# pletzer/nemoflux

Measured on AMD Instinct MI355X. Metric: edge-flux integrals/sec, higher is better.
Workload: dtype f64

## Files before the change

### nemoflux_amd/csrc/nf_capi_field.hip

```cpp
#include "nf_capi.h"

using namespace nf;

static int g_batch_steps = 1;
static long g_batch_cellsteps = 32l << 20;
static int g_partial_full = 0;
static int g_use_graph = 1;
static int g_inner_signed = 1;
static int g_k3_pairs = 1;
static long g_knob_version = 0;

namespace nf {
int field_tuning_set(const char *name, int value)
{
    ++g_knob_version;
    if (!strcmp(name, "batch_steps")) {
        g_batch_steps = value;
        return NF_OK;
    }
    if (!strcmp(name, "batch_cellsteps_m")) {
        if (!(value >= 0 && value <= 2047)) return -1;
        g_batch_cellsteps = (long)value << 20;
        return NF_OK;
    }
    if (!strcmp(name, "partial_step_planes")) {
        g_partial_full = value != 0;
        return NF_OK;
    }
    if (!strcmp(name, "graph")) {
        g_use_graph = value != 0;
        return NF_OK;
    }
    if (!strcmp(name, "pass_inner_signed")) {
        g_inner_signed = value != 0;
        return NF_OK;
    }
    if (!strcmp(name, "pass_k3_pairs")) {
        g_k3_pairs = value != 0;
        return NF_OK;
    }
    return -1;
}
}

struct nf_field {
    hipStream_t stream = nullptr;
    long ny = 0, nx = 0, ncell = 0, nz = 0, nt = 0;
    struct Geometry {
        DevArray<double> xy, arc4, arcE, arcN;
        DevArray<unsigned long long> box;
        DevArray<double> iV;
        DevArray<double> abs;
        DevArray<double> aos;
        DevArray<double> uv2;
        DevArray<double> tr_planes;
        DevArray<unsigned long long> maxbits;
        DevArray<double> iVb, absb, scratchb;
        DevArray<int> zr;
        long batch_steps = 0, batch_version = -1;
    } geo;
    double box[4] = {0, 0, 0, 0};
    DevArray<double> thick;
    const void *u = nullptr, *v = nullptr;
    int uv_dtype = NF_F64, uv_on_device = 1;
    double fill = std::numeric_limits<double>::quiet_NaN();
    double fill2 = std::numeric_limits<double>::quiet_NaN();
    DevArray<char> stage_u, stage_v;
    int sverdrup = 0;
    long s_begin = 0, s_end = -1;
    int compact = 0;
    bool derived_stale = false;
    std::vector<std::vector<double>> polylines;
    std::vector<int> poly_cc;
    std::vector<int> tr_off;
    WeightSet ws;
    bool weights_built = false;
    int skip_unsupported = 0;
// ... 103 lines not shown
}

static int field_timed_k3_end(nf_field *f)
{
    if (!f->timing || f->ev_used == 0 || f->ev_dropped) return NF_OK;
    auto &t = f->ev[f->ev_used - 1];
    NF_HIP(hipEventRecord(t.e2, f->stream));
    t.has_k3 = true;
    return NF_OK;
}

static int field_ensure_derived(nf_field *f)
{
    if (!f->derived_stale) return NF_OK;
    NF_TRY(launch_expand_planes(f->geo.iV.get(), f->geo.abs.get(), f->ncell, f->ny, f->nx, f->stream));
    f->derived_stale = false;
    return NF_OK;
}

static int field_row_length(const nf_field *f) { return f->ws.nseg + (int)f->polylines.size(); }

struct StepForm {
    bool inner = false;
    bool to_uv2 = false;
};

static int field_step_input(nf_field *f, long t, int z0, int z1, const void **ut, const void **vt)
{
    const size_t es = elem_size(f->uv_dtype);
    const size_t step_bytes = (size_t)f->nz * f->ncell * es;
    if (f->uv_on_device) {
        *ut = (const char *)f->u + (size_t)t * step_bytes;
        *vt = (const char *)f->v + (size_t)t * step_bytes;
        return NF_OK;
    }
    NF_TRY(f->stage_u.reserve(step_bytes));
    NF_TRY(f->stage_v.reserve(step_bytes));
    const size_t off = (size_t)z0 * f->ncell * es, len = (size_t)(z1 - z0) * f->ncell * es;
    NF_HIP(hipMemcpyAsync(f->stage_u.get() + off, (const char *)f->u + (size_t)t * step_bytes + off, len,
                          hipMemcpyHostToDevice, f->stream));
    NF_HIP(hipMemcpyAsync(f->stage_v.get() + off, (const char *)f->v + (size_t)t * step_bytes + off, len,
                          hipMemcpyHostToDevice, f->stream));
    *ut = f->stage_u.get();
    *vt = f->stage_v.get();
    return NF_OK;
}

// ... 11 lines not shown
        if (row_dev && rowlen > 0) NF_HIP(hipMemsetAsync(row_dev, 0, sizeof(double) * rowlen, f->stream));
        return NF_OK;
    }
    const int z0 = (int)(lo - t * f->nz), z1 = (int)(hi - t * f->nz);
    const void *ut, *vt;
    NF_TRY(field_step_input(f, t, z0, z1, &ut, &vt));
    FluxArgs a{};
    a.u = ut;
    a.v = vt;
    a.dtype = f->uv_dtype;
    a.ncell = f->ncell;
    a.ny = f->ny;
    a.nx = f->nx;
    a.z0 = z0;
    a.z1 = z1;
    a.thickness = f->thick.get();
    a.arcE = f->geo.arcE.get();
    a.arcN = f->geo.arcN.get();
    a.fill = f->fill;
    a.fill2 = f->fill2;
    a.scale = kEarthRadiusSv / 1.e6;
    a.sverdrup = f->sverdrup;
    a.iV = f->geo.iV.get();
    if (form.to_uv2) a.iV = f->geo.uv2.get() - f->ncell;
    a.absU = f->geo.abs.get();
    a.absV = f->geo.abs.get() + f->ncell;
    a.maxbits = f->geo.maxbits.get();
    const bool partial = (z0 > 0 || z1 < (int)f->nz) && !g_partial_full;
    a.signed_only = (f->compact || partial || form.inner) && flux_supports_signed_only(a);
    NF_REQUIRE(!form.to_uv2 || a.signed_only, NF_ERR_STATE, "compute: a step into the second planes must be signed-only");
    if (!form.to_uv2) f->derived_stale = a.signed_only != 0;
    if (f->timing) {
        NF_TRY(field_timed_flux(f, a));
    } else {
        NF_TRY(launch_flux(a, f->stream));
    }
    if (row_dev && rowlen > 0 && !form.to_uv2) {
        NF_REQUIRE(f->weights_built, NF_ERR_STATE, "compute: build_weights first");
        NF_TRY(launch_integral(f->ws, f->geo.iV.get(), f->ncell, 2, f->nx, f->tr_off_dev.get(), (int)f->polylines.size(),
                               f->scratch.get(), row_dev, f->stream));
        NF_TRY(field_timed_k3_end(f));
    }
    return NF_OK;
}

static int field_profile_async(nf_field *f, long t, double *prof_dev)
{
    NF_REQUIRE(f->geo.arcE.get() && f->thick.get() && f->u && f->v, NF_ERR_STATE,
               "compute_profile: set_bounds, set_thickness and set_uv first");
    NF_REQUIRE(f->weights_built, NF_ERR_STATE, "compute_profile: build_weights first");
    NF_REQUIRE(t >= 0 && t < f->nt, NF_ERR_ARG, "compute_profile: time index out of range");
    const int rowlen = field_row_length(f);
    if (rowlen == 0) return NF_OK;
    const long s_end = f->s_end < 0 ? f->nt * f->nz : f->s_end;
    long lo = t * f->nz, hi = (t + 1) * f->nz;
    if (lo < f->s_begin) lo = f->s_begin;
    if (hi > s_end) hi = s_end;
    if (hi < lo) hi = lo;
    const int z0 = (int)(lo - t * f->nz), z1 = (int)(hi - t * f->nz);
    if (z0 > 0) NF_HIP(hipMemsetAsync(prof_dev, 0, sizeof(double) * rowlen * (size_t)z0, f->stream));
// ... 61 lines not shown
    a.dtype = f->uv_dtype;
    a.ncell = f->ncell;
    a.ny = f->ny;
    a.nx = f->nx;
    a.z0 = z0;
    a.z1 = z1;
    a.thickness = f->thick.get();
    a.arcE = f->geo.arcE.get();
    a.arcN = f->geo.arcN.get();
    a.fill = f->fill;
    a.fill2 = f->fill2;
    a.tfill = f->tau_fill;
    a.tfill2 = f->tau_fill2;
    a.ref = f->tau_ref;
    a.wrap_x = f->tau_wrap;
    a.scale = kEarthRadiusSv / 1.e6;
    a.sverdrup = f->sverdrup;
    a.planes = f->geo.tr_planes.get();
    NF_TRY(launch_tracer_flux(a, f->stream));
    return launch_integral(f->ws, f->geo.tr_planes.get() - f->ncell, f->ncell, 2, f->nx, f->tr_off_dev.get(),
                           (int)f->polylines.size(), f->scratch.get(), row_dev, f->stream);
}

static int field_pair_async(nf_field *f, long t, double *rows_dev, bool last)
{
    const int rowlen = field_row_length(f);
    StepForm first, second;
    first.inner = first.to_uv2 = true;
    second.inner = g_inner_signed && !last;
    NF_TRY(field_step_async(f, t, nullptr, first));
    NF_TRY(field_step_async(f, t + 1, nullptr, second));
    NF_TRY(launch_integral_pair(f->ws, f->geo.uv2.get(), f->geo.iV.get() + f->ncell, f->ncell, f->nx, f->tr_off_dev.get(),
                                (int)f->polylines.size(), f->scratch.get(), rows_dev + (size_t)t * rowlen, rowlen, f->stream));
    NF_TRY(field_timed_k3_end(f));
    return NF_OK;
}

static long batch_cell_steps() { return g_batch_cellsteps; }

static bool field_can_batch(const nf_field *f)
{
    return g_batch_steps && f->uv_on_device && f->nt >= 2 && f->nt < 65536 && f->nt * f->ncell <= batch_cell_steps() &&
           f->ncell <= (1l << 20) && f->weights_built;
}

static bool field_pass_pairs(const nf_field *f)
{
    if (!g_k3_pairs || integral_uses_edges() || !f->geo.uv2.get() || !f->weights_built) return false;
    const size_t step_bytes = (size_t)f->nz * f->ncell * elem_size(f->uv_dtype);
    FluxArgs a{};
    a.u = f->uv_on_device ? f->u : nullptr;
    a.v = f->uv_on_device ? f->v : nullptr;
    a.dtype = f->uv_dtype;
    a.ncell = f->ncell;
    return flux_supports_signed_only(a) && (!f->uv_on_device || step_bytes % 16 == 0);
}

static int field_prepare_pass(nf_field *f)
{
    if (!g_k3_pairs || integral_uses_edges() || f->geo.uv2.get() || !f->geo.iV.get() || f->nz <= 0) return NF_OK;
    const long total = f->nt * f->nz;
    const long s_end = f->s_end < 0 ? total : std::min(f->s_end, total);
    if (s_end - std::min(f->s_begin, s_end) < 2 * f->nz) return NF_OK;
    NF_TRY(f->geo.uv2.alloc((size_t)f->ncell * 2));
    return NF_OK;
}

static int field_all_steps_direct(nf_field *f, double *rows_dev)
{
    const int rowlen = field_row_length(f);
    const long total = f->nt * f->nz;
    const long s_end = f->s_end < 0 ? total : std::min(f->s_end, total);
    const long s_begin = std::min(f->s_begin, s_end);
    const long ta = s_end > s_begin ? s_begin / f->nz : 0;
    const long tb = s_end > s_begin ? (s_end - 1) / f->nz + 1 : 0;
    if (rowlen > 0) {
        if (ta > 0) NF_HIP(hipMemsetAsync(rows_dev, 0, sizeof(double) * rowlen * (size_t)ta, f->stream));
        if (tb < f->nt)
            NF_HIP(hipMemsetAsync(rows_dev + (size_t)tb * rowlen, 0, sizeof(double) * rowlen * (size_t)(f->nt - tb),
                                  f->stream));
    }
    const long wa = (ta < tb && s_begin > ta * f->nz) ? ta + 1 : ta;
    const long wb = std::max(wa, (ta < tb && s_end < tb * f->nz) ? tb - 1 : tb);
    const bool pairs = field_pass_pairs(f) && rowlen > 0;
    const long pa = pairs ? wa + (wb - wa) % 2 : wb;
    for (long t = ta; t < tb;) {
        const bool last = t + 1 == tb;
        if (t >= pa && t + 1 < wb) {
            NF_TRY(field_pair_async(f, t, rows_dev, t + 2 == tb));
            t += 2;
        } else {
            StepForm form;
            form.inner = g_inner_signed && !last;
            NF_TRY(field_step_async(f, t, rows_dev + (size_t)t * rowlen, form));
            t += 1;
        }
    }
    return NF_OK;
}

static int field_all_steps_batched(nf_field *f, double *rows_dev)
{
    const int rowlen = field_row_length(f);
    const size_t n = (size_t)f->ncell;
    nf_field::Geometry &g = f->geo;
    if (g.batch_steps != f->nt) {
        NF_TRY(g.iVb.alloc(n * 4 * f->nt));
        NF_TRY(g.absb.alloc(n * 2 * f->nt));
        NF_TRY(g.zr.alloc((size_t)2 * f->nt));
        NF_HIP(hipMemsetAsync(g.iVb.get(), 0, sizeof(double) * n * 4 * f->nt, f->stream));
        g.batch_steps = f->nt;
        g.batch_version = -1;
// ... 691 lines not shown
```

### nemoflux_amd/csrc/nf_capi_util.hip

```cpp
#include "nf_capi.h"

namespace nf {

static thread_local std::string g_err;
void set_error(const std::string &msg) { g_err = msg; }
int hip_fail(hipError_t e, const char *what, const char *file, int line)
{
    char buf[512];
    snprintf(buf, sizeof buf, "HIP error %d (%s) in %s at %s:%d", (int)e, hipGetErrorString(e), what, file, line);
    g_err = buf;
    return (e == hipErrorNoDevice || e == hipErrorInvalidDevice) ? NF_ERR_NO_DEVICE : NF_ERR_HIP;
}

int require_device()
{
    int n = 0;
    hipError_t e = hipGetDeviceCount(&n);
    if (e != hipSuccess || n <= 0) {
        set_error("no usable AMD GPU (hipGetDeviceCount); nemoflux_amd has no CPU fallback");
        return NF_ERR_NO_DEVICE;
    }
    return NF_OK;
}

// ... 82 lines not shown
    NF_HIP(hipMemcpy(dev, host, bytes, hipMemcpyHostToDevice));
    return NF_OK;
}
NF_API_CATCH
int nf_memcpy_d2h(void *host, const void *dev, size_t bytes)
try {
    NF_NEED_DEVICE();
    NF_HIP(hipMemcpy(host, dev, bytes, hipMemcpyDeviceToHost));
    return NF_OK;
}
NF_API_CATCH
int nf_memset(void *dev, int value, size_t bytes)
try {
    NF_NEED_DEVICE();
    NF_HIP(hipMemset(dev, value, bytes));
    return NF_OK;
}
NF_API_CATCH
int nf_tuning_set(const char *name, int value)
try {
    NF_REQUIRE(name, NF_ERR_ARG, "nf_tuning_set: null name");
    if (!strcmp(name, "batch_cellsteps_m"))
        NF_REQUIRE(value >= 0 && value <= 2047, NF_ERR_ARG, "nf_tuning_set: batch_cellsteps_m must be in [0, 2047]");
    if (field_tuning_set(name, value) == NF_OK) return NF_OK;
    if (!strcmp(name, "edge_weights")) {
        integral_use_edges(value);
        return NF_OK;
    }
    if (!strcmp(name, "datagen_rows")) {
        datagen_use_rows(value);
        return NF_OK;
    }
    int rc = tuning_set(name, value);
    NF_REQUIRE(rc == NF_OK, NF_ERR_ARG, std::string("nf_tuning_set: unknown knob ") + name);
    return NF_OK;
}
NF_API_CATCH
int nf_release_scratch(void)
try {
    weights_trim_scratch();
    return NF_OK;
}
NF_API_CATCH
int nf_synchronize(void)
try {
    NF_NEED_DEVICE();
// ... 98 lines not shown
```

### nemoflux_amd/csrc/nf_common.h

```cpp
#pragma once
#include <hip/hip_runtime.h>
#include <cstdint>
#include <cstdio>
#include <string>
#include <cmath>
#include <initializer_list>
#include <mutex>
#include <vector>

#include "../../include/nemoflux_amd.h"

namespace nf {

constexpr int kWave = 64;
constexpr int kBlock = 256;
constexpr int kXcds = 8;
constexpr double kDeg2Rad = 3.14159265358979323846 / 180.0;
constexpr double kEarthRadiusSv = 6371000.0;

void set_error(const std::string &msg);
int hip_fail(hipError_t e, const char *what, const char *file, int line);

#define NF_HIP(call)                                                   \
    do {                                                               \
// ... 87 lines not shown
double box_key_to_double(unsigned long long k);

struct StepBatch {
    int nsteps = 0;
    long in_stride = 0;
    const int *zr = nullptr;
};

struct FluxArgs {
    const void *u, *v;
    int dtype;
    long ncell, ny, nx;
    int z0, z1;
    const double *thickness;
    const double *arcE, *arcN;
    double fill;
    double fill2 = __builtin_nan("");
    double scale;
    int sverdrup;
    double *iV, *absU, *absV;
    unsigned long long *maxbits;
    StepBatch batch;
    int signed_only = 0;
    hipEvent_t mid_event = nullptr;
    bool *mid_recorded = nullptr;
};
int launch_flux(const FluxArgs &a, hipStream_t s);
bool flux_supports_signed_only(const FluxArgs &a);
int launch_expand_planes(double *iV, double *absUV, long ncell, long ny, long nx, hipStream_t s);
int tuning_set(const char *name, int value);
long tuning_version();
int launch_planes_to_aos(const double *planes, long ncell, double *aos, hipStream_t s);

template <typename T>
class DevArray {
public:
    DevArray() = default;
    DevArray(const DevArray &) = delete;
    DevArray &operator=(const DevArray &) = delete;
    DevArray(DevArray &&o) noexcept : p_(o.p_), n_(o.n_) { o.p_ = nullptr, o.n_ = 0; }
    DevArray &operator=(DevArray &&o) noexcept
    {
        if (this != &o) {
            reset();
            p_ = o.p_, n_ = o.n_;
            o.p_ = nullptr, o.n_ = 0;
        }
        return *this;
    }
    ~DevArray() { reset(); }
    int alloc(size_t n)
// ... 47 lines not shown
};
int fold_weights(WeightSet *ws, long ncell, long nx, hipStream_t s);
int weights_to_host(const WeightSet &ws, int64_t *cell_edge, double *weight, int *seg);
struct Box4;
struct LocatorBoxes {
    std::vector<DevArray<Box4>> level;
    std::vector<long> count;
    const double *xy = nullptr;
    long ncell = 0;
    double period = -1.0;
    std::mutex mtx;
    void release();
};
int build_weights(const double *xy, long ncell, const double *segs_host, const int *seg_cc_host, int nseg,
                  double periodX, WeightSet *out, hipStream_t s, int skip_unsupported = 0, int overlap_warn = 0,
                  LocatorBoxes *boxes = nullptr, long row_length = 0);
void weights_trim_scratch();

void integral_use_edges(int on);
int integral_uses_edges();
int launch_integral(const WeightSet &ws, const double *data, long ncell, int planes, long nx,
                    const int *tr_offsets_dev, int ntransect, double *scratch, double *row, hipStream_t s,
                    int nsteps = 1, long data_stride = 0, long row_stride = 0, const int *rec_cells = nullptr);
int launch_integral_pair(const WeightSet &ws, const double *uvA, const double *uvB, long ncell, long nx,
                         const int *tr_offsets_dev, int ntransect, double *scratch, double *row, long row_stride,
                         hipStream_t s);

constexpr int kProfileChunk = 8;
struct ProfileArgs {
    const WeightSet *ws = nullptr;
    const void *u = nullptr, *v = nullptr;
    int dtype = NF_F64;
    long ncell = 0, nx = 0;
    int z0 = 0, z1 = 0;
    const double *thickness = nullptr, *arcE = nullptr, *arcN = nullptr;
    double fill = __builtin_nan(""), fill2 = __builtin_nan("");
    double scale = 1.0;
    int sverdrup = 0;
    const int *tr_offsets_dev = nullptr;
    int ntransect = 0;
    long row_length = 0;
    double *scratch = nullptr;
    size_t scratch_len = 0;
    double *prof = nullptr;
};
int launch_profile(const ProfileArgs &a, hipStream_t s);

struct TracerArgs {
// ... 30 lines not shown
```

### nemoflux_amd/csrc/nf_flux.hip

```cpp
#include <cstring>

#include "nf_common.h"

namespace nf {

template <typename T, int VEC> struct vec_t;
typedef double dvec2 __attribute__((ext_vector_type(2)));
typedef float fvec4 __attribute__((ext_vector_type(4)));
template <> struct vec_t<double, 2> { using type = dvec2; };
template <> struct vec_t<float, 4> { using type = fvec4; };
template <> struct vec_t<double, 1> { using type = double; };
template <> struct vec_t<float, 1> { using type = float; };

template <typename T, int VEC> struct Lanes {
    T x[VEC];
};

template <typename T, int VEC, bool NT>
__device__ inline Lanes<T, VEC> load_cells(const T *p)
{
    using V = typename vec_t<T, VEC>::type;
    Lanes<T, VEC> r;
    V v = NT ? __builtin_nontemporal_load(reinterpret_cast<const V *>(p)) : *reinterpret_cast<const V *>(p);
    __builtin_memcpy(&r, &v, sizeof(V));
// ... 59 lines not shown
        }
        if (i0 + VEC <= nx) {
            if (j0 + 1 < ny) {
                const bool al = (nx & 1u) == 0;
#pragma unroll
                for (int k = 0; k < VEC; k += 2) store2<NTS>(p0 + c0 + nx + k, eV[k], eV[k + 1], al);
            }
#pragma unroll
            for (int k = 0; k < VEC; ++k) store1<NTS>(p3 + ((i0 + k + 1 < nx) ? c0 + k + 1 : c0 + k + 1 - nx), eU[k]);
        } else {
#pragma unroll
            for (int k = 0; k < VEC; ++k) {
                const long c = c0 + k;
                const unsigned j = (unsigned)(c / nx);
                const unsigned i = (unsigned)(c - (long)j * nx);
                if (j + 1 < ny) store1<NTS>(p0 + c + nx, eV[k]);
                store1<NTS>(p3 + ((i + 1 < nx) ? c + 1 : c + 1 - nx), eU[k]);
            }
        }
    }
}

constexpr int kFormSignedOnly = 16;
constexpr int kFormNestedLoads = 128;
constexpr int kFormTwoFills = 256;
#ifdef NF_TUNING_BUILD
constexpr int kDiagNoStores = 1, kDiagNoFix = 2, kDiagNoMax = 4, kDiagNoArc = 8, kDiagInterleaved = 32, kDiagPlainStores = 64;
#else
constexpr int kDiagNoStores = 0, kDiagNoFix = 0, kDiagNoMax = 0, kDiagNoArc = 0, kDiagInterleaved = 0, kDiagPlainStores = 0;
#endif

template <typename T, int VEC, int UZ, bool NT, int BLOCK, int CH, int FORM = 0>
__global__ __launch_bounds__(BLOCK) void k_flux(const T *__restrict__ u, const T *__restrict__ v, long ncell,
                                                unsigned ny, unsigned nx, int z0, int z1,
                                                const double *__restrict__ thickness,
                                                const double *__restrict__ arcE, const double *__restrict__ arcN,
                                                T fill, double scale, int sverdrup, double *__restrict__ iV,
                                                double *__restrict__ absUV, unsigned long long *maxbits,
                                                unsigned ntiles, int xcd_map, StepBatch sb, T fill2)
{
#ifndef NF_TUNING_BUILD
    static_assert((FORM & ~(kFormSignedOnly | kFormNestedLoads | kFormTwoFills)) == 0, "diagnostic forms exist only in tuning builds");
#endif
    const unsigned tile = xcd_map ? xcd_tile(blockIdx.x, gridDim.x) : blockIdx.x;
    if (sb.zr) {
        const long tb = blockIdx.y;
        u += tb * sb.in_stride;
        v += tb * sb.in_stride;
        iV += tb * 4 * ncell;
        absUV += tb * 2 * ncell;
        z0 = sb.zr[2 * tb];
        z1 = sb.zr[2 * tb + 1];
    }
    double tmax = 0.0;
    if (tile < ntiles) {
        const long base = (long)tile * BLOCK * VEC * CH + (long)threadIdx.x * VEC;
        constexpr long kChunk = (long)BLOCK * VEC;
        bool on[CH];
        double accU[CH][VEC], accV[CH][VEC];
#pragma unroll
        for (int q = 0; q < CH; ++q) {
            on[q] = base + q * kChunk < ncell;
#pragma unroll
            for (int k = 0; k < VEC; ++k) accU[q][k] = accV[q][k] = 0.0;
        }
// ... 40 lines not shown
                                    accV[q][k] = fma(th, (FORM & kDiagNoFix) ? (double)lv[r][q].x[k] : fixed<T>(lv[r][q].x[k], fill), accV[q][k]);
                                }
                            }
                        }
                }
            pu += (long)UZ * ncell;
            pv += (long)UZ * ncell;
        }
#pragma unroll
        for (int q = 0; q < CH; ++q)
            if (on[q]) {
                const long c0 = base + q * kChunk;
                double eU[VEC], eV[VEC];
#pragma unroll
                for (int k = 0; k < VEC; ++k) {
                    eU[k] = +accU[q][k] * ((FORM & kDiagNoArc) ? 1.5 : arcE[c0 + k]);
                    eV[k] = -accV[q][k] * ((FORM & kDiagNoArc) ? 1.5 : arcN[c0 + k]);
                    if (sverdrup) {
                        eU[k] *= scale;
                        eV[k] *= scale;
                    }
                    tmax = fmax(tmax, fmax(fabs(eU[k]), fabs(eV[k])));
                }
                if (FORM & kDiagInterleaved) {
#pragma unroll
                    for (int k = 0; k < VEC; ++k) store2<true>(iV + 2 * (c0 + k), eU[k], eV[k], true);
                } else if (FORM & kFormSignedOnly) {
#pragma unroll
                    for (int k = 0; k < VEC; k += 2) {
                        store2<true>(iV + ncell + c0 + k, eU[k], eU[k + 1], true);
                        store2<true>(iV + 2 * ncell + c0 + k, eV[k], eV[k + 1], true);
                    }
                } else if (!(FORM & kDiagNoStores)) store_cells<VEC, !(FORM & kDiagPlainStores)>(c0, eU, eV, ncell, ny, nx, iV, absUV);
            }
    }
    for (int o = 32; o > 0; o >>= 1) tmax = fmax(tmax, __shfl_xor(tmax, o, kWave));
    if ((threadIdx.x & (kWave - 1)) == 0 && tmax > 0.0 && !(FORM & kDiagNoMax)) {
        unsigned long long b;
        __builtin_memcpy(&b, &tmax, 8);
        if (b > __hip_atomic_load(maxbits, __ATOMIC_RELAXED, __HIP_MEMORY_SCOPE_AGENT)) atomicMax(maxbits, b);
    }
}

template <typename T, int VEC, int UZ, bool SIGNED_ONLY, bool TWO_FILLS, bool WSHIFT = false>
__global__ __launch_bounds__(256) void k_flux_field(const T *__restrict__ u, const T *__restrict__ v, long ncell,
                                                    unsigned ny, unsigned nx, int z0, int z1,
                                                    const double *__restrict__ thickness,
// ... 198 lines not shown
    const unsigned ntiles = (unsigned)((a.ncell + per_tile - 1) / per_tile);
    const int xcd_map = g_xcd_map;
    const unsigned grid = xcd_map ? xcd_grid(ntiles) : ntiles;
    hipLaunchKernelGGL((k_flux_field<T, VEC, UZ, SIGNED_ONLY, TWO_FILLS, WSHIFT>), dim3(grid, (unsigned)(a.batch.zr ? a.batch.nsteps : 1), 2),
                       dim3(256), 0, s, (const T *)a.u, (const T *)a.v, a.ncell, (unsigned)a.ny, (unsigned)a.nx, a.z0, a.z1,
                       a.thickness, a.arcE, a.arcN, (T)a.fill, a.scale, a.sverdrup, a.iV, a.absU, a.maxbits, ntiles, xcd_map,
                       a.batch, (T)a.fill2);
    NF_HIP(hipGetLastError());
    return NF_OK;
}

template <typename T, int VEC>
static int launch_flux_field(const FluxArgs &a, hipStream_t s)
{
    constexpr int kLevels = sizeof(T) == 8 ? 10 : 16;
    const bool two = (T)a.fill2 == (T)a.fill2 && !((T)a.fill2 == (T)a.fill);
    if (a.signed_only)
        return two ? launch_flux_field_t<T, VEC, kLevels, true, true>(a, s) : launch_flux_field_t<T, VEC, kLevels, true, false>(a, s);
    if (g_west_shift && VEC > 1)
        return two ? launch_flux_field_t<T, VEC, kLevels, false, true, true>(a, s) : launch_flux_field_t<T, VEC, kLevels, false, false, true>(a, s);
    return two ? launch_flux_field_t<T, VEC, kLevels, false, true>(a, s) : launch_flux_field_t<T, VEC, kLevels, false, false>(a, s);
}

template <typename T, int VEC>
static int launch_flux_v(const FluxArgs &a, hipStream_t s)
{
    const int variant = a.batch.zr ? 0 : g_variant;
    if (variant == 0) {
        const long waves = (a.ncell / VEC + kWave - 1) / kWave;
        const bool split = g_field_split < 0 ? (!a.batch.zr && waves < kFieldSplitWaves) : g_field_split != 0;
        if (split) return launch_flux_field<T, VEC>(a, s);
    }
    const bool two = (T)a.fill2 == (T)a.fill2 && !((T)a.fill2 == (T)a.fill);
    if (a.signed_only) {
        NF_REQUIRE(VEC > 1 && !a.batch.zr, NF_ERR_STATE, "flux: the compact mode needs 16-byte aligned fields, an even cell count and one step per launch");
        if (two) return launch_flux_t<T, VEC, (sizeof(T) == 8 ? 10 : 8), true, 256, 1, kFormSignedOnly | kFormTwoFills>(a, s);
        return launch_flux_t<T, VEC, (sizeof(T) == 8 ? 10 : 8), true, 256, 1, kFormSignedOnly>(a, s);
    }
    if (VEC == 1) {
        if (two) return launch_flux_t<T, VEC, 8, true, 256, 1, kFormTwoFills>(a, s);
        return launch_flux_t<T, VEC, 8, true, 256, 1>(a, s);
    }
    if (two) {
        constexpr int kLevels = sizeof(T) == 8 ? 10 : 8;
        if (a.batch.zr || sizeof(T) == 8) return launch_flux_t<T, VEC, kLevels, true, 256, 1, kFormTwoFills>(a, s);
        const int rc = launch_flux_t<T, VEC, kLevels, true, 256, 1, kFormSignedOnly | kFormTwoFills>(a, s);
        if (rc != NF_OK) return rc;
        if (a.mid_event) {
            NF_HIP(hipEventRecord(a.mid_event, s));
            if (a.mid_recorded) *a.mid_recorded = true;
        }
        return launch_expand_planes(a.iV, a.absU, a.ncell, a.ny, a.nx, s);
    }
    switch (variant) {
#ifdef NF_TUNING_BUILD
        case 3: return launch_flux_t<T, VEC, 4, true, 256, 1>(a, s);
        case 4: return launch_flux_t<T, VEC, 4, true, 256, 2>(a, s);
        case 11: return launch_flux_t<T, VEC, 10, false, 256, 1>(a, s);
        case 12: return launch_flux_t<T, VEC, 8, true, 256, 1>(a, s);
        case 14: return launch_flux_t<T, VEC, 16, true, 256, 1>(a, s);
        case 13: return launch_flux_t<T, VEC, 10, true, 256, 1, kDiagPlainStores>(a, s);
        case 40: return launch_flux_ww<T, VEC, 2>(a, s);
        case 21: return launch_flux_t<T, VEC, 10, true, 256, 1, kDiagNoStores>(a, s);
        case 28: return launch_flux_t<T, VEC, 10, true, 256, 1, kFormSignedOnly>(a, s);
        case 29: return launch_flux_t<T, VEC, 10, true, 256, 1, kDiagInterleaved>(a, s);
        case 45: return launch_flux_ww<T, VEC, 2, 2>(a, s);
        case 6: {
            const int rc = launch_flux_t<T, VEC, (sizeof(T) == 8 ? 10 : 8), true, 256, 1, kFormSignedOnly | kFormNestedLoads>(a, s);
            return rc != NF_OK ? rc : launch_expand_planes(a.iV, a.absU, a.ncell, a.ny, a.nx, s);
        }
#endif
        case 5:
        default: {
            constexpr int kLevels = sizeof(T) == 8 ? 10 : 8;
            const bool fused = a.batch.zr || ((sizeof(T) == 8) != (variant == 5));
            if (fused) return launch_flux_t<T, VEC, kLevels, true, 256, 1>(a, s);
            const int rc = launch_flux_t<T, VEC, kLevels, true, 256, 1, kFormSignedOnly>(a, s);
            if (rc != NF_OK) return rc;
            if (a.mid_event) {
                NF_HIP(hipEventRecord(a.mid_event, s));
                if (a.mid_recorded) *a.mid_recorded = true;
            }
            return launch_expand_planes(a.iV, a.absU, a.ncell, a.ny, a.nx, s);
        }
    }
}

bool flux_supports_signed_only(const FluxArgs &a)
{
    const bool al16 = ((uintptr_t)a.u % 16 == 0) && ((uintptr_t)a.v % 16 == 0);
    return al16 && !a.batch.zr && a.ncell % (a.dtype == NF_F32 ? 4 : 2) == 0;
}

int launch_flux(const FluxArgs &a, hipStream_t s)
{
    NF_REQUIRE(a.ncell > 0 && a.ncell == a.ny * a.nx && a.ncell < (1l << 31), NF_ERR_ARG, "flux: bad grid sizes");
    NF_REQUIRE(a.batch.zr || (a.z1 > a.z0 && a.z0 >= 0), NF_ERR_ARG, "flux: empty z range");
    NF_REQUIRE(!a.batch.zr || (a.batch.nsteps > 0 && a.batch.nsteps < 65536), NF_ERR_ARG, "flux: bad step batch");
    NF_REQUIRE(a.absV == a.absU + a.ncell, NF_ERR_ARG, "flux: abs planes must be contiguous");
    const bool al16 = ((uintptr_t)a.u % 16 == 0) && ((uintptr_t)a.v % 16 == 0);
    if (a.dtype == NF_F64) {
        if (al16 && a.ncell % 2 == 0) return launch_flux_v<double, 2>(a, s);
        return launch_flux_v<double, 1>(a, s);
    } else if (a.dtype == NF_F32) {
        if (al16 && a.ncell % 4 == 0) return launch_flux_v<float, 4>(a, s);
        return launch_flux_v<float, 1>(a, s);
    }
    NF_REQUIRE(false, NF_ERR_ARG, "flux: dtype must be NF_F64 or NF_F32");
}

__global__ __launch_bounds__(kBlock) void k_planes_to_aos(const double *__restrict__ planes, long ncell,
                                                          double *__restrict__ aos)
{
    long c = (long)blockIdx.x * kBlock + threadIdx.x;
    if (c < ncell) {
        double2 *o = reinterpret_cast<double2 *>(aos + 4 * c);
// ... 14 lines not shown
```

### nemoflux_amd/csrc/nf_integral.hip

```cpp
#include "nf_common.h"

namespace nf {

__global__ __launch_bounds__(kBlock) void k_gather_segscan(const int *__restrict__ cell,
                                                           const double *__restrict__ w4,
                                                           const int *__restrict__ seg, long n,
                                                           const double *__restrict__ data, long ncell,
                                                           int planes, unsigned nx, double *__restrict__ runsum,
                                                           long data_stride)
{
    data += (long)blockIdx.y * data_stride;
    runsum += (long)blockIdx.y * n;
    const long k = (long)blockIdx.x * kBlock + threadIdx.x;
    const int lane = threadIdx.x & (kWave - 1);
    double val = 0.0;
    int key = -1;
    if (k < n) {
        typedef double dvec2 __attribute__((ext_vector_type(2)));
        const long c = __builtin_nontemporal_load(cell + k);
        const dvec2 *pw = reinterpret_cast<const dvec2 *>(w4 + 4 * k);
        const dvec2 wa = __builtin_nontemporal_load(pw), wb = __builtin_nontemporal_load(pw + 1);
        double d0, d1, d2, d3;
        if (planes == 2) {
            const unsigned j = (unsigned)(c / nx), i = (unsigned)(c - (long)j * nx);
// ... 5 lines not shown
        } else if (planes) {
            d0 = data[c];
            d1 = data[ncell + c];
            d2 = data[2 * ncell + c];
            d3 = data[3 * ncell + c];
        } else {
            const double2 *pd = reinterpret_cast<const double2 *>(data + 4 * c);
            const double2 da = pd[0], db = pd[1];
            d0 = da.x; d1 = da.y; d2 = db.x; d3 = db.y;
        }
        val = ((wa.x * d0 + wa.y * d1) + wb.x * d2) + wb.y * d3;
        key = __builtin_nontemporal_load(seg + k);
    }
#pragma unroll
    for (int o = 1; o < kWave; o <<= 1) {
        const double pv = __shfl_up(val, o, kWave);
        const int pk = __shfl_up(key, o, kWave);
        if (lane >= o && pk == key) val += pv;
    }
    const int nk = __shfl_down(key, 1, kWave);
    if (k < n && (lane == kWave - 1 || k == n - 1 || nk != key)) runsum[k] = val;
}

__global__ __launch_bounds__(kBlock) void k_gather_segscan_pair(const int *__restrict__ cell, const double *__restrict__ w4,
                                                                const int *__restrict__ seg, long n,
                                                                const double *__restrict__ uvA,
                                                                const double *__restrict__ uvB, long ncell, unsigned nx,
                                                                double *__restrict__ runsum)
{
    const long k = (long)blockIdx.x * kBlock + threadIdx.x;
    const int lane = threadIdx.x & (kWave - 1);
    double va = 0.0, vb = 0.0;
    int key = -1;
    if (k < n) {
        typedef double dvec2 __attribute__((ext_vector_type(2)));
        const long c = __builtin_nontemporal_load(cell + k);
        const dvec2 *pw = reinterpret_cast<const dvec2 *>(w4 + 4 * k);
        const dvec2 wa = __builtin_nontemporal_load(pw), wb = __builtin_nontemporal_load(pw + 1);
        const unsigned j = (unsigned)(c / nx), i = (unsigned)(c - (long)j * nx);
        const long cw = i > 0 ? c - 1 : c - 1 + nx;
        {
            const double *eU = uvA, *eV = uvA + ncell;
            const double d1 = eU[c], d2 = eV[c], d0 = j > 0 ? eV[c - nx] : 0.0, d3 = eU[cw];
            va = ((wa.x * d0 + wa.y * d1) + wb.x * d2) + wb.y * d3;
        }
        {
            const double *eU = uvB, *eV = uvB + ncell;
            const double d1 = eU[c], d2 = eV[c], d0 = j > 0 ? eV[c - nx] : 0.0, d3 = eU[cw];
            vb = ((wa.x * d0 + wa.y * d1) + wb.x * d2) + wb.y * d3;
        }
        key = __builtin_nontemporal_load(seg + k);
    }
#pragma unroll
    for (int o = 1; o < kWave; o <<= 1) {
        const double pa = __shfl_up(va, o, kWave), pb = __shfl_up(vb, o, kWave);
        const int pk = __shfl_up(key, o, kWave);
        if (lane >= o && pk == key) {
            va += pa;
            vb += pb;
        }
    }
    const int nk = __shfl_down(key, 1, kWave);
    if (k < n && (lane == kWave - 1 || k == n - 1 || nk != key)) {
        runsum[k] = va;
        runsum[n + k] = vb;
    }
}

__global__ __launch_bounds__(kBlock) void k_gather_edges(const WeightSet::EdgeEntry *__restrict__ ent, long n,
                                                         const double *__restrict__ data, long ncell,
                                                         double *__restrict__ runsum, long data_stride)
{
    data += (long)blockIdx.y * data_stride + ncell;
// ... 41 lines not shown
        }
    }
    for (int o = 32; o > 0; o >>= 1) acc += __shfl_xor(acc, o, kWave);
    if (lane == 0) row[s] = acc;
}

__global__ __launch_bounds__(kBlock) void k_finalize_tr(const int *__restrict__ tr_off, int ntransect, int nseg,
                                                        double *__restrict__ row, long row_stride)
{
    row += (long)blockIdx.y * row_stride;
    const int p = (blockIdx.x * kBlock + threadIdx.x) / kWave;
    const int lane = threadIdx.x & (kWave - 1);
    if (p >= ntransect) return;
    double part = 0.0;
    for (int s = tr_off[p] + lane; s < tr_off[p + 1]; s += kWave) part += row[s];
    for (int o = 32; o > 0; o >>= 1) part += __shfl_xor(part, o, kWave);
    if (lane == 0) row[nseg + p] = part;
}

static int g_use_edges = 0;
void integral_use_edges(int on) { g_use_edges = on; }
int integral_uses_edges() { return g_use_edges; }

int launch_integral(const WeightSet &ws, const double *data, long ncell, int planes, long nx,
                    const int *tr_offsets_dev, int ntransect, double *scratch, double *row, hipStream_t s, int nsteps,
                    long data_stride, long row_stride, const int *rec_cells)
{
    const unsigned ny = (unsigned)(nsteps > 1 ? nsteps : 1);
    if (planes == 2 && ws.ent_start.get() && g_use_edges) {
        if (ws.nent > 0)
            hipLaunchKernelGGL(k_gather_edges, dim3((unsigned)((ws.nent + kBlock - 1) / kBlock), ny), dim3(kBlock), 0, s,
                               ws.ent.get(), ws.nent, data, ncell, scratch, data_stride);
        if (ws.nseg > 0) {
            const unsigned nb = (unsigned)(((long)ws.nseg * kWave + kBlock - 1) / kBlock);
            hipLaunchKernelGGL(k_finalize_seg, dim3(nb, ny), dim3(kBlock), 0, s, scratch, ws.ent_start.get(), ws.nseg, row,
                               ws.nent, row_stride);
        }
        if (ntransect > 0) {
            const unsigned nb = (unsigned)(((long)ntransect * kWave + kBlock - 1) / kBlock);
            hipLaunchKernelGGL(k_finalize_tr, dim3(nb, ny), dim3(kBlock), 0, s, tr_offsets_dev, ntransect, ws.nseg, row,
                               row_stride);
        }
        NF_HIP(hipGetLastError());
        return NF_OK;
    }
    if (ws.nrec > 0) {
        hipLaunchKernelGGL(k_gather_segscan, dim3((unsigned)((ws.nrec + kBlock - 1) / kBlock), ny), dim3(kBlock), 0, s,
                           rec_cells ? rec_cells : ws.cell.get(), ws.w4.get(), ws.seg.get(), ws.nrec, data, ncell, planes,
                           (unsigned)(nx > 0 ? nx : 1), scratch, data_stride);
    }
    if (ws.nseg > 0) {
        const unsigned nb = (unsigned)(((long)ws.nseg * kWave + kBlock - 1) / kBlock);
        hipLaunchKernelGGL(k_finalize_seg, dim3(nb, ny), dim3(kBlock), 0, s, scratch, ws.seg_start.get(), ws.nseg, row,
                           ws.nrec, row_stride);
    }
    if (ntransect > 0) {
        const unsigned nb = (unsigned)(((long)ntransect * kWave + kBlock - 1) / kBlock);
        hipLaunchKernelGGL(k_finalize_tr, dim3(nb, ny), dim3(kBlock), 0, s, tr_offsets_dev, ntransect, ws.nseg, row,
                           row_stride);
    }
    NF_HIP(hipGetLastError());
    return NF_OK;
}

int launch_integral_pair(const WeightSet &ws, const double *uvA, const double *uvB, long ncell, long nx,
                         const int *tr_offsets_dev, int ntransect, double *scratch, double *row, long row_stride,
                         hipStream_t s)
{
    if (ws.nrec > 0)
        hipLaunchKernelGGL(k_gather_segscan_pair, dim3((unsigned)((ws.nrec + kBlock - 1) / kBlock)), dim3(kBlock), 0, s,
                           ws.cell.get(), ws.w4.get(), ws.seg.get(), ws.nrec, uvA, uvB, ncell, (unsigned)(nx > 0 ? nx : 1),
                           scratch);
    if (ws.nseg > 0) {
        const unsigned nb = (unsigned)(((long)ws.nseg * kWave + kBlock - 1) / kBlock);
        hipLaunchKernelGGL(k_finalize_seg, dim3(nb, 2), dim3(kBlock), 0, s, scratch, ws.seg_start.get(), ws.nseg, row,
                           ws.nrec, row_stride);
    }
    if (ntransect > 0) {
        const unsigned nb = (unsigned)(((long)ntransect * kWave + kBlock - 1) / kBlock);
        hipLaunchKernelGGL(k_finalize_tr, dim3(nb, 2), dim3(kBlock), 0, s, tr_offsets_dev, ntransect, ws.nseg, row,
                           row_stride);
    }
    NF_HIP(hipGetLastError());
    return NF_OK;
}

template <typename T>
__device__ inline double profile_fixed(T x, T fill, T fill2, bool two)
{
    return (x != x || x == fill || (two && x == fill2)) ? 0.0 : (double)x;
}

template <typename T, int LZ>
__global__ __launch_bounds__(kBlock) void k_profile_segscan(const int *__restrict__ cell, const double *__restrict__ w4,
                                                            const int *__restrict__ seg, long n, const T *__restrict__ u,
// ... 112 lines not shown
```

Measured before the change: 379.6 billion.

## Store paired-step edge fluxes interleaved so the integral gathers U,V with one vector load

In the two-step pass, the flux kernel now writes each step's signed edge values as interleaved (U,V) pairs into side buffers (uv2, plus a new uv3 for the second step). The paired gather kernel is templated on the layout so it reads U and V of a cell with one 16-byte load. The aim is fewer scattered memory transactions in the gather that follows each flux step. In exchange it adds an extra buffer, more kernel template variants, and a different flux kernel variant whose own store speed may differ.

```diff
diff --git a/nemoflux_amd/csrc/nf_capi_field.hip b/nemoflux_amd/csrc/nf_capi_field.hip
--- a/nemoflux_amd/csrc/nf_capi_field.hip
+++ b/nemoflux_amd/csrc/nf_capi_field.hip
@@ -8,6 +8,7 @@
 static int g_use_graph = 1;
 static int g_inner_signed = 1;
 static int g_k3_pairs = 1;
+static int g_interleaved = 1;
 static long g_knob_version = 0;
 
 namespace nf {
@@ -37,6 +38,11 @@
     }
     if (!strcmp(name, "pass_k3_pairs")) {
         g_k3_pairs = value != 0;
+        return NF_OK;
+    }
+    if (!strcmp(name, "pass_interleaved")) {
+        if (value != 0 && value != 1) return -1;
+        g_interleaved = value;
         return NF_OK;
     }
     return -1;
@@ -53,6 +59,7 @@
         DevArray<double> abs;
         DevArray<double> aos;
         DevArray<double> uv2;
+        DevArray<double> uv3;
         DevArray<double> tr_planes;
         DevArray<unsigned long long> maxbits;
         DevArray<double> iVb, absb, scratchb;
@@ -202,7 +209,8 @@
 
 struct StepForm {
     bool inner = false;
-    bool to_uv2 = false;
+    double *side = nullptr;
+    bool interleaved = false;
 };
 
 static int field_step_input(nf_field *f, long t, int z0, int z1, const void **ut, const void **vt)
@@ -260,20 +268,24 @@
     a.scale = kEarthRadiusSv / 1.e6;
     a.sverdrup = f->sverdrup;
     a.iV = f->geo.iV.get();
-    if (form.to_uv2) a.iV = f->geo.uv2.get() - f->ncell;
+    if (form.side) a.iV = form.interleaved ? form.side : form.side - f->ncell;
     a.absU = f->geo.abs.get();
     a.absV = f->geo.abs.get() + f->ncell;
     a.maxbits = f->geo.maxbits.get();
     const bool partial = (z0 > 0 || z1 < (int)f->nz) && !g_partial_full;
     a.signed_only = (f->compact || partial || form.inner) && flux_supports_signed_only(a);
-    NF_REQUIRE(!form.to_uv2 || a.signed_only, NF_ERR_STATE, "compute: a step into the second planes must be signed-only");
-    if (!form.to_uv2) f->derived_stale = a.signed_only != 0;
+    NF_REQUIRE(!form.side || a.signed_only, NF_ERR_STATE, "compute: a step into the second planes must be signed-only");
+    if (form.interleaved) {
+        NF_REQUIRE(form.side && flux_supports_interleaved(a), NF_ERR_STATE, "compute: no interleaved form for this step");
+        a.interleaved = 1;
+    }
+    if (!form.side) f->derived_stale = a.signed_only != 0;
     if (f->timing) {
         NF_TRY(field_timed_flux(f, a));
     } else {
         NF_TRY(launch_flux(a, f->stream));
     }
-    if (row_dev && rowlen > 0 && !form.to_uv2) {
+    if (row_dev && rowlen > 0 && !form.side) {
         NF_REQUIRE(f->weights_built, NF_ERR_STATE, "compute: build_weights first");
         NF_TRY(launch_integral(f->ws, f->geo.iV.get(), f->ncell, 2, f->nx, f->tr_off_dev.get(), (int)f->polylines.size(),
                                f->scratch.get(), row_dev, f->stream));
@@ -381,16 +393,24 @@
                            (int)f->polylines.size(), f->scratch.get(), row_dev, f->stream);
 }
 
-static int field_pair_async(nf_field *f, long t, double *rows_dev, bool last)
+static int field_pair_async(nf_field *f, long t, double *rows_dev, bool last, bool inter)
 {
     const int rowlen = field_row_length(f);
     StepForm first, second;
-    first.inner = first.to_uv2 = true;
+    first.inner = true;
+    first.side = f->geo.uv2.get();
+    first.interleaved = inter;
     second.inner = g_inner_signed && !last;
+    if (second.inner && inter && f->geo.uv3.get()) {
+        second.side = f->geo.uv3.get();
+        second.interleaved = true;
+    }
     NF_TRY(field_step_async(f, t, nullptr, first));
     NF_TRY(field_step_async(f, t + 1, nullptr, second));
-    NF_TRY(launch_integral_pair(f->ws, f->geo.uv2.get(), f->geo.iV.get() + f->ncell, f->ncell, f->nx, f->tr_off_dev.get(),
-                                (int)f->polylines.size(), f->scratch.get(), rows_dev + (size_t)t * rowlen, rowlen, f->stream));
+    const double *uvB = second.side ? second.side : f->geo.iV.get() + f->ncell;
+    NF_TRY(launch_integral_pair(f->ws, first.side, first.interleaved, uvB, second.interleaved, f->ncell, f->nx,
+                                f->tr_off_dev.get(), (int)f->polylines.size(), f->scratch.get(), rows_dev + (size_t)t * rowlen,
+                                rowlen, f->stream));
     NF_TRY(field_timed_k3_end(f));
     return NF_OK;
 }
@@ -415,13 +435,27 @@
     return flux_supports_signed_only(a) && (!f->uv_on_device || step_bytes % 16 == 0);
 }
 
+static bool field_pass_interleaved(const nf_field *f)
+{
+    if (!g_interleaved || f->uv_dtype != NF_F64) return false;
+    FluxArgs a{};
+    a.u = f->uv_on_device ? f->u : nullptr;
+    a.v = f->uv_on_device ? f->v : nullptr;
+    a.dtype = f->uv_dtype;
+    a.ncell = f->ncell;
+    return flux_supports_interleaved(a);
+}
+
 static int field_prepare_pass(nf_field *f)
 {
-    if (!g_k3_pairs || integral_uses_edges() || f->geo.uv2.get() || !f->geo.iV.get() || f->nz <= 0) return NF_OK;
+    if (!g_k3_pairs || integral_uses_edges() || !f->geo.iV.get() || f->nz <= 0) return NF_OK;
     const long total = f->nt * f->nz;
     const long s_end = f->s_end < 0 ? total : std::min(f->s_end, total);
-    if (s_end - std::min(f->s_begin, s_end) < 2 * f->nz) return NF_OK;
-    NF_TRY(f->geo.uv2.alloc((size_t)f->ncell * 2));
+    const long owned = s_end - std::min(f->s_begin, s_end);
+    if (owned < 2 * f->nz) return NF_OK;
+    if (!f->geo.uv2.get()) NF_TRY(f->geo.uv2.alloc((size_t)f->ncell * 2));
+    if (!f->geo.uv3.get() && g_interleaved && owned >= 4 * f->nz && field_pass_interleaved(f))
+        NF_TRY(f->geo.uv3.alloc((size_t)f->ncell * 2));
     return NF_OK;
 }
 
@@ -442,11 +476,12 @@
     const long wa = (ta < tb && s_begin > ta * f->nz) ? ta + 1 : ta;
     const long wb = std::max(wa, (ta < tb && s_end < tb * f->nz) ? tb - 1 : tb);
     const bool pairs = field_pass_pairs(f) && rowlen > 0;
+    const bool inter = pairs && field_pass_interleaved(f);
     const long pa = pairs ? wa + (wb - wa) % 2 : wb;
     for (long t = ta; t < tb;) {
         const bool last = t + 1 == tb;
         if (t >= pa && t + 1 < wb) {
-            NF_TRY(field_pair_async(f, t, rows_dev, t + 2 == tb));
+            NF_TRY(field_pair_async(f, t, rows_dev, t + 2 == tb, inter));
             t += 2;
         } else {
             StepForm form;
diff --git a/nemoflux_amd/csrc/nf_capi_util.hip b/nemoflux_amd/csrc/nf_capi_util.hip
--- a/nemoflux_amd/csrc/nf_capi_util.hip
+++ b/nemoflux_amd/csrc/nf_capi_util.hip
@@ -128,6 +128,8 @@
     NF_REQUIRE(name, NF_ERR_ARG, "nf_tuning_set: null name");
     if (!strcmp(name, "batch_cellsteps_m"))
         NF_REQUIRE(value >= 0 && value <= 2047, NF_ERR_ARG, "nf_tuning_set: batch_cellsteps_m must be in [0, 2047]");
+    if (!strcmp(name, "pass_interleaved"))
+        NF_REQUIRE(value == 0 || value == 1, NF_ERR_ARG, "nf_tuning_set: pass_interleaved must be 0 or 1");
     if (field_tuning_set(name, value) == NF_OK) return NF_OK;
     if (!strcmp(name, "edge_weights")) {
         integral_use_edges(value);
diff --git a/nemoflux_amd/csrc/nf_common.h b/nemoflux_amd/csrc/nf_common.h
--- a/nemoflux_amd/csrc/nf_common.h
+++ b/nemoflux_amd/csrc/nf_common.h
@@ -133,11 +133,13 @@
     unsigned long long *maxbits;
     StepBatch batch;
     int signed_only = 0;
+    int interleaved = 0;
     hipEvent_t mid_event = nullptr;
     bool *mid_recorded = nullptr;
 };
 int launch_flux(const FluxArgs &a, hipStream_t s);
 bool flux_supports_signed_only(const FluxArgs &a);
+bool flux_supports_interleaved(const FluxArgs &a);
 int launch_expand_planes(double *iV, double *absUV, long ncell, long ny, long nx, hipStream_t s);
 int tuning_set(const char *name, int value);
 long tuning_version();
@@ -231,8 +233,8 @@
 int launch_integral(const WeightSet &ws, const double *data, long ncell, int planes, long nx,
                     const int *tr_offsets_dev, int ntransect, double *scratch, double *row, hipStream_t s,
                     int nsteps = 1, long data_stride = 0, long row_stride = 0, const int *rec_cells = nullptr);
-int launch_integral_pair(const WeightSet &ws, const double *uvA, const double *uvB, long ncell, long nx,
-                         const int *tr_offsets_dev, int ntransect, double *scratch, double *row, long row_stride,
+int launch_integral_pair(const WeightSet &ws, const double *uvA, bool interA, const double *uvB, bool interB, long ncell,
+                         long nx, const int *tr_offsets_dev, int ntransect, double *scratch, double *row, long row_stride,
                          hipStream_t s);
 
 constexpr int kProfileChunk = 8;
diff --git a/nemoflux_amd/csrc/nf_flux.hip b/nemoflux_amd/csrc/nf_flux.hip
--- a/nemoflux_amd/csrc/nf_flux.hip
+++ b/nemoflux_amd/csrc/nf_flux.hip
@@ -105,12 +105,13 @@
 }
 
 constexpr int kFormSignedOnly = 16;
+constexpr int kFormInterleaved = 32;
 constexpr int kFormNestedLoads = 128;
 constexpr int kFormTwoFills = 256;
 #ifdef NF_TUNING_BUILD
-constexpr int kDiagNoStores = 1, kDiagNoFix = 2, kDiagNoMax = 4, kDiagNoArc = 8, kDiagInterleaved = 32, kDiagPlainStores = 64;
+constexpr int kDiagNoStores = 1, kDiagNoFix = 2, kDiagNoMax = 4, kDiagNoArc = 8, kDiagPlainStores = 64;
 #else
-constexpr int kDiagNoStores = 0, kDiagNoFix = 0, kDiagNoMax = 0, kDiagNoArc = 0, kDiagInterleaved = 0, kDiagPlainStores = 0;
+constexpr int kDiagNoStores = 0, kDiagNoFix = 0, kDiagNoMax = 0, kDiagNoArc = 0, kDiagPlainStores = 0;
 #endif
 
 template <typename T, int VEC, int UZ, bool NT, int BLOCK, int CH, int FORM = 0>
@@ -123,7 +124,8 @@
                                                 unsigned ntiles, int xcd_map, StepBatch sb, T fill2)
 {
 #ifndef NF_TUNING_BUILD
-    static_assert((FORM & ~(kFormSignedOnly | kFormNestedLoads | kFormTwoFills)) == 0, "diagnostic forms exist only in tuning builds");
+    static_assert((FORM & ~(kFormSignedOnly | kFormInterleaved | kFormNestedLoads | kFormTwoFills)) == 0,
+                  "diagnostic forms exist only in tuning builds");
 #endif
     const unsigned tile = xcd_map ? xcd_tile(blockIdx.x, gridDim.x) : blockIdx.x;
     if (sb.zr) {
@@ -210,7 +212,7 @@
                     }
                     tmax = fmax(tmax, fmax(fabs(eU[k]), fabs(eV[k])));
                 }
-                if (FORM & kDiagInterleaved) {
+                if (FORM & kFormInterleaved) {
 #pragma unroll
                     for (int k = 0; k < VEC; ++k) store2<true>(iV + 2 * (c0 + k), eU[k], eV[k], true);
                 } else if (FORM & kFormSignedOnly) {
@@ -455,13 +457,25 @@
     return two ? launch_flux_field_t<T, VEC, kLevels, false, true>(a, s) : launch_flux_field_t<T, VEC, kLevels, false, false>(a, s);
 }
 
+static bool flux_field_split(long ncell, int vec)
+{
+    const long waves = (ncell / vec + kWave - 1) / kWave;
+    return g_field_split < 0 ? waves < kFieldSplitWaves : g_field_split != 0;
+}
+
 template <typename T, int VEC>
 static int launch_flux_v(const FluxArgs &a, hipStream_t s)
 {
     const int variant = a.batch.zr ? 0 : g_variant;
+    if (a.interleaved) {
+        NF_REQUIRE(VEC > 1 && !a.batch.zr, NF_ERR_STATE, "flux: the interleaved form needs the 16-byte vector path");
+        const bool two = (T)a.fill2 == (T)a.fill2 && !((T)a.fill2 == (T)a.fill);
+        constexpr int kLevels = sizeof(T) == 8 ? 10 : 8;
+        if (two) return launch_flux_t<T, VEC, kLevels, true, 256, 1, kFormInterleaved | kFormTwoFills>(a, s);
+        return launch_flux_t<T, VEC, kLevels, true, 256, 1, kFormInterleaved>(a, s);
+    }
     if (variant == 0) {
-        const long waves = (a.ncell / VEC + kWave - 1) / kWave;
-        const bool split = g_field_split < 0 ? (!a.batch.zr && waves < kFieldSplitWaves) : g_field_split != 0;
+        const bool split = g_field_split < 0 ? (!a.batch.zr && flux_field_split(a.ncell, VEC)) : g_field_split != 0;
         if (split) return launch_flux_field<T, VEC>(a, s);
     }
     const bool two = (T)a.fill2 == (T)a.fill2 && !((T)a.fill2 == (T)a.fill);
@@ -496,7 +510,7 @@
         case 40: return launch_flux_ww<T, VEC, 2>(a, s);
         case 21: return launch_flux_t<T, VEC, 10, true, 256, 1, kDiagNoStores>(a, s);
         case 28: return launch_flux_t<T, VEC, 10, true, 256, 1, kFormSignedOnly>(a, s);
-        case 29: return launch_flux_t<T, VEC, 10, true, 256, 1, kDiagInterleaved>(a, s);
+        case 29: return launch_flux_t<T, VEC, 10, true, 256, 1, kFormInterleaved>(a, s);
         case 45: return launch_flux_ww<T, VEC, 2, 2>(a, s);
         case 6: {
             const int rc = launch_flux_t<T, VEC, (sizeof(T) == 8 ? 10 : 8), true, 256, 1, kFormSignedOnly | kFormNestedLoads>(a, s);
@@ -525,6 +539,11 @@
     return al16 && !a.batch.zr && a.ncell % (a.dtype == NF_F32 ? 4 : 2) == 0;
 }
 
+bool flux_supports_interleaved(const FluxArgs &a)
+{
+    return flux_supports_signed_only(a) && !flux_field_split(a.ncell, a.dtype == NF_F32 ? 4 : 2);
+}
+
 int launch_flux(const FluxArgs &a, hipStream_t s)
 {
     NF_REQUIRE(a.ncell > 0 && a.ncell == a.ny * a.nx && a.ncell < (1l << 31), NF_ERR_ARG, "flux: bad grid sizes");
diff --git a/nemoflux_amd/csrc/nf_integral.hip b/nemoflux_amd/csrc/nf_integral.hip
--- a/nemoflux_amd/csrc/nf_integral.hip
+++ b/nemoflux_amd/csrc/nf_integral.hip
@@ -51,6 +51,32 @@
     if (k < n && (lane == kWave - 1 || k == n - 1 || nk != key)) runsum[k] = val;
 }
 
+typedef double dvec2 __attribute__((ext_vector_type(2)));
+
+constexpr int kUvPlanes = 0, kUvInterleaved = 1;
+
+template <int LAYOUT>
+__device__ inline double pair_value(const double *__restrict__ uv, long ncell, long c, long cw, long cs, bool south, dvec2 wa,
+                                    dvec2 wb)
+{
+    double d0, d1, d2, d3;
+    if (LAYOUT == kUvInterleaved) {
+        const dvec2 ec = reinterpret_cast<const dvec2 *>(uv)[c];
+        d1 = ec.x;
+        d2 = ec.y;
+        d0 = south ? uv[2 * cs + 1] : 0.0;
+        d3 = uv[2 * cw];
+    } else {
+        const double *eU = uv, *eV = uv + ncell;
+        d1 = eU[c];
+        d2 = eV[c];
+        d0 = south ? eV[cs] : 0.0;
+        d3 = eU[cw];
+    }
+    return ((wa.x * d0 + wa.y * d1) + wb.x * d2) + wb.y * d3;
+}
+
+template <int LA, int LB>
 __global__ __launch_bounds__(kBlock) void k_gather_segscan_pair(const int *__restrict__ cell, const double *__restrict__ w4,
                                                                 const int *__restrict__ seg, long n,
                                                                 const double *__restrict__ uvA,
@@ -62,22 +88,13 @@
     double va = 0.0, vb = 0.0;
     int key = -1;
     if (k < n) {
-        typedef double dvec2 __attribute__((ext_vector_type(2)));
         const long c = __builtin_nontemporal_load(cell + k);
         const dvec2 *pw = reinterpret_cast<const dvec2 *>(w4 + 4 * k);
         const dvec2 wa = __builtin_nontemporal_load(pw), wb = __builtin_nontemporal_load(pw + 1);
         const unsigned j = (unsigned)(c / nx), i = (unsigned)(c - (long)j * nx);
         const long cw = i > 0 ? c - 1 : c - 1 + nx;
-        {
-            const double *eU = uvA, *eV = uvA + ncell;
-            const double d1 = eU[c], d2 = eV[c], d0 = j > 0 ? eV[c - nx] : 0.0, d3 = eU[cw];
-            va = ((wa.x * d0 + wa.y * d1) + wb.x * d2) + wb.y * d3;
-        }
-        {
-            const double *eU = uvB, *eV = uvB + ncell;
-            const double d1 = eU[c], d2 = eV[c], d0 = j > 0 ? eV[c - nx] : 0.0, d3 = eU[cw];
-            vb = ((wa.x * d0 + wa.y * d1) + wb.x * d2) + wb.y * d3;
-        }
+        va = pair_value<LA>(uvA, ncell, c, cw, c - nx, j > 0, wa, wb);
+        vb = pair_value<LB>(uvB, ncell, c, cw, c - nx, j > 0, wa, wb);
         key = __builtin_nontemporal_load(seg + k);
     }
 #pragma unroll
@@ -165,6 +182,14 @@
 void integral_use_edges(int on) { g_use_edges = on; }
 int integral_uses_edges() { return g_use_edges; }
 
+template <int LA, int LB>
+static void launch_pair_l(const WeightSet &ws, const double *uvA, const double *uvB, long ncell, unsigned nx, double *scratch,
+                          hipStream_t s)
+{
+    hipLaunchKernelGGL((k_gather_segscan_pair<LA, LB>), dim3((unsigned)((ws.nrec + kBlock - 1) / kBlock)), dim3(kBlock), 0, s,
+                       ws.cell.get(), ws.w4.get(), ws.seg.get(), ws.nrec, uvA, uvB, ncell, nx, scratch);
+}
+
 int launch_integral(const WeightSet &ws, const double *data, long ncell, int planes, long nx,
                     const int *tr_offsets_dev, int ntransect, double *scratch, double *row, hipStream_t s, int nsteps,
                     long data_stride, long row_stride, const int *rec_cells)
@@ -206,14 +231,17 @@
     return NF_OK;
 }
 
-int launch_integral_pair(const WeightSet &ws, const double *uvA, const double *uvB, long ncell, long nx,
-                         const int *tr_offsets_dev, int ntransect, double *scratch, double *row, long row_stride,
+int launch_integral_pair(const WeightSet &ws, const double *uvA, bool interA, const double *uvB, bool interB, long ncell,
+                         long nx, const int *tr_offsets_dev, int ntransect, double *scratch, double *row, long row_stride,
                          hipStream_t s)
 {
-    if (ws.nrec > 0)
-        hipLaunchKernelGGL(k_gather_segscan_pair, dim3((unsigned)((ws.nrec + kBlock - 1) / kBlock)), dim3(kBlock), 0, s,
-                           ws.cell.get(), ws.w4.get(), ws.seg.get(), ws.nrec, uvA, uvB, ncell, (unsigned)(nx > 0 ? nx : 1),
-                           scratch);
+    if (ws.nrec > 0) {
+        const unsigned ux = (unsigned)(nx > 0 ? nx : 1);
+        if (interA && interB) launch_pair_l<kUvInterleaved, kUvInterleaved>(ws, uvA, uvB, ncell, ux, scratch, s);
+        else if (interA) launch_pair_l<kUvInterleaved, kUvPlanes>(ws, uvA, uvB, ncell, ux, scratch, s);
+        else if (interB) launch_pair_l<kUvPlanes, kUvInterleaved>(ws, uvA, uvB, ncell, ux, scratch, s);
+        else launch_pair_l<kUvPlanes, kUvPlanes>(ws, uvA, uvB, ncell, ux, scratch, s);
+    }
     if (ws.nseg > 0) {
         const unsigned nb = (unsigned)(((long)ws.nseg * kWave + kBlock - 1) / kBlock);
         hipLaunchKernelGGL(k_finalize_seg, dim3(nb, 2), dim3(kBlock), 0, s, scratch, ws.seg_start.get(), ws.nseg, row,
```

Result: faster. 387.1 billion, median of 6 (+2.0%).
